# wafgo/rt-depth-map

Measured on AMD Instinct MI355X. Metric: stereo-pairs/sec, 1280x720 d=64 9x9 SAD, higher is better.
Workload: dtype u8

## Files before the change

rt-depth-map_amd/csrc/api_bm.hip:

```cpp
#include "rtdm_handles.h"

using namespace rtdm;

void rtdm_bm_default_params(rtdm_bm_params* p, int numDisparities)
{
    if (!p) return;
    p->preFilterCap = 31; p->blockSize = 13; p->minDisparity = 0; p->numDisparities = numDisparities;
    p->textureThreshold = 10; p->uniquenessRatio = 10; p->speckleWindowSize = 100; p->speckleRange = 32;
    p->disp12MaxDiff = 1; p->legacy_right_clamp = 0;
}

static int validate_params(const rtdm_bm_params& p)
{
    if (p.preFilterCap < 1 || p.preFilterCap > 63) return RTDM_ERR_BAD_PARAM;
    if (p.blockSize < 5 || p.blockSize > 255 || (p.blockSize & 1) == 0) return RTDM_ERR_BAD_PARAM;
    if (p.numDisparities <= 0 || p.numDisparities % 16 != 0) return RTDM_ERR_BAD_PARAM;
    if (p.textureThreshold < 0 || p.uniquenessRatio < 0) return RTDM_ERR_BAD_PARAM;
    if (p.minDisparity < -2047 || (long)p.minDisparity + p.numDisparities > 2047) return RTDM_ERR_BAD_PARAM;
    if (p.legacy_right_clamp != 0 && p.legacy_right_clamp != 1) return RTDM_ERR_BAD_PARAM;
    return RTDM_OK;
}

int rtdm_bm_create(const rtdm_bm_params* params, int max_width, int max_height, int max_batch,
                   int device, rtdm_bm** out)
{
    if (!params || !out) return RTDM_ERR_NULL;
    *out = nullptr;
    int rc = validate_params(*params);
    if (rc) return rc;
    if (max_width <= 0 || max_height <= 0 || max_batch <= 0 || max_width > 32767 || max_height > 32767)
        return RTDM_ERR_BAD_SIZE;
    if ((long)max_batch * max_width * max_height >= (1L << 31)) return RTDM_ERR_BAD_SIZE;
    if (max_width > 4096) return RTDM_ERR_UNSUPPORTED;
    rc = use_device(device);
    if (rc) return rc;
    rtdm_bm* bm = new (std::nothrow) rtdm_bm();
    if (!bm) return RTDM_ERR_NOMEM;
    bm->p = *params; bm->prefilter_type = RTDM_PREFILTER_XSOBEL; bm->prefilter_size = 9;
    bm->maxW = max_width; bm->maxH = max_height; bm->maxB = max_batch; bm->device = device;
    bm->ppitch = ((size_t)max_width + 63) & ~(size_t)63;
    const size_t plane = bm->ppitch * max_height * (size_t)max_batch;
    const size_t px = bm_ws(max_width) * max_height * max_batch;
    AllocList& m = bm->mem;
    m.err = hipStreamCreateWithFlags(&bm->stream, hipStreamNonBlocking);
    const size_t plane_al = (plane + 1024 + 255) & ~(size_t)255;
    if (m.dev(&bm->dLp, 2 * plane_al)) bm->dRp = bm->dLp + plane_al;
    m.dev(&bm->dInL, plane); m.dev(&bm->dInR, plane); m.dev(&bm->dOut, px * sizeof(int16_t));
    m.dev(&bm->dCost, px * sizeof(int32_t)); m.dev(&bm->dLabel, px * sizeof(int32_t)); m.dev(&bm->dSize, px * sizeof(int32_t));
    m.dev(&bm->dRuns, px * sizeof(uint32_t)); m.dev(&bm->dHead, px * sizeof(int16_t));
    m.dev(&bm->dMask, (size_t)max_width * max_height); m.dev(&bm->dDepth, depth_scratch_bytes(RTDM_MAX_REGIONS, max_height));
    const size_t hplanes = 2 * bm->ppitch * (size_t)max_height, hpx = bm_ws(max_width) * max_height;
    m.host(&bm->hStage, hplanes + hpx * (sizeof(int16_t) + 1) + 1024);
    if (bm->hStage) { bm->hD = (int16_t*)(bm->hStage + hplanes); bm->hM = (uint8_t*)(bm->hD + hpx); }
    m.dev(&bm->dRowCnt, (size_t)max_batch * max_height * sizeof(int32_t));
    hipError_t e = m.err;
    const auto new_event = [&e](hipEvent_t* ev) { if (e == hipSuccess) e = hipEventCreateWithFlags(ev, hipEventDisableTiming); };
    const auto new_stream = [&e](hipStream_t* q) { if (e == hipSuccess) e = hipStreamCreateWithFlags(q, hipStreamNonBlocking); };
    for (auto& ev : bm->evBand) new_event(&ev);
    new_stream(&bm->sIn); new_stream(&bm->sOut);
    for (int k = 0; k < 2; ++k) { new_event(&bm->evH2D[k]); new_event(&bm->evComp[k]); new_event(&bm->evD2H[k]); }
    new_stream(&bm->sSpare[0]); new_stream(&bm->sBorder); new_stream(&bm->sSpare[1]);
    new_event(&bm->evFork); new_event(&bm->evJoin);
    if (e != hipSuccess) { rtdm_bm_destroy(bm); return create_failed("rtdm_bm_create", e); }
    *out = bm;
    return RTDM_OK;
}

void rtdm_bm_destroy(rtdm_bm* bm)
{
    if (!bm) return;
    (void)hipSetDevice(bm->device);
    if (bm->stream) (void)hipStreamSynchronize(bm->stream);
    if (bm->sBorder) { (void)hipStreamSynchronize(bm->sBorder); (void)hipStreamDestroy(bm->sBorder); }
    for (auto& q : bm->sSpare) if (q) (void)hipStreamDestroy(q);
    for (hipEvent_t e : {bm->evFork, bm->evJoin, bm->evBand[0], bm->evBand[1]}) if (e) (void)hipEventDestroy(e);
    if (bm->sIn) { (void)hipStreamSynchronize(bm->sIn); (void)hipStreamDestroy(bm->sIn); }
    if (bm->sOut) { (void)hipStreamSynchronize(bm->sOut); (void)hipStreamDestroy(bm->sOut); }
    for (int k = 0; k < 2; ++k)
        for (hipEvent_t e : {bm->evH2D[k], bm->evComp[k], bm->evD2H[k]}) if (e) (void)hipEventDestroy(e);
    for (auto& ev : bm->pending) { (void)hipEventDestroy(ev.a); (void)hipEventDestroy(ev.b); }
    bm->mem.release();
    if (bm->stream) (void)hipStreamDestroy(bm->stream);
    delete bm;
}

int rtdm_bm_set_roi(rtdm_bm* bm, int which, int x, int y, int width, int height)
{
    if (!bm) return RTDM_ERR_NULL;
    if (which != 1 && which != 2) return RTDM_ERR_BAD_PARAM;
    int* r = which == 1 ? bm->roi1 : bm->roi2;
    r[0] = x; r[1] = y; r[2] = width; r[3] = height;
    return RTDM_OK;
}

int rtdm_bm_get_params(const rtdm_bm* bm, rtdm_bm_params* out)
{
    if (!bm || !out) return RTDM_ERR_NULL;
    *out = bm->p;
    return RTDM_OK;
}

int rtdm_bm_set_prefilter(rtdm_bm* bm, int preFilterType, int preFilterSize)
{
    if (!bm) return RTDM_ERR_NULL;
    if (preFilterType != RTDM_PREFILTER_NORMALIZED_RESPONSE && preFilterType != RTDM_PREFILTER_XSOBEL) return RTDM_ERR_BAD_PARAM;
    if (preFilterSize < 5 || preFilterSize > 255 || (preFilterSize & 1) == 0) return RTDM_ERR_BAD_PARAM;
    bm->prefilter_type = preFilterType; bm->prefilter_size = preFilterSize;
    return RTDM_OK;
}

int rtdm_bm_get_prefilter(const rtdm_bm* bm, int* preFilterType, int* preFilterSize)
{
    if (!bm || !preFilterType || !preFilterSize) return RTDM_ERR_NULL;
    *preFilterType = bm->prefilter_type; *preFilterSize = bm->prefilter_size;
    return RTDM_OK;
}

static bool make_geom(const rtdm_bm* bm, int W, int H, BMGeom* g)
{
    const rtdm_bm_params& p = bm->p;
    g->W = W; g->H = H; g->Ws = (W + 7) & ~7; g->D = p.numDisparities; g->minD = p.minDisparity;
    g->w = p.blockSize; g->r = p.blockSize / 2;
    g->cap = p.preFilterCap; g->tex = p.textureThreshold; g->uniq = p.uniquenessRatio;
    g->lofs = std::max(g->D - 1 + g->minD, 0);
    g->rofs = -std::min(g->D - 1 + g->minD, 0);
    g->width1 = W - g->rofs - g->D + 1;
    g->filtered = (g->minD - 1) * 16;
    g->want_cost = p.disp12MaxDiff >= 0;
    g->cost16 = 2L * p.preFilterCap * p.blockSize * p.blockSize < 65536;
    g->mask_cols = p.disp12MaxDiff < 0;
    g->legacy = p.legacy_right_clamp;
    int r1[4] = {0, 0, W, H}, r2[4] = {0, 0, W, H};
    if (bm->roi1[2] > 0 && bm->roi1[3] > 0) std::copy(bm->roi1, bm->roi1 + 4, r1);
    if (bm->roi2[2] > 0 && bm->roi2[3] > 0) std::copy(bm->roi2, bm->roi2 + 4, r2);
    const int maxD = g->minD + g->D - 1;
    int xmin = std::max(r1[0], r2[0] + maxD) + g->r;
    int xmax = std::min(r1[0] + r1[2], r2[0] + r2[2] - g->minD) - g->r;
    int ymin = std::max(r1[1], r2[1]) + g->r;
    int ymax = std::min(r1[1] + r1[3], r2[1] + r2[3]) - g->r;
    xmin = std::max(xmin, 0); xmax = std::min(xmax, W);
    ymin = std::max(ymin, g->r); ymax = std::min(ymax, H - g->r);
    g->vx0 = xmin; g->vx1 = xmax; g->vy0 = ymin; g->vy1 = ymax;
    const int reach = (p.disp12MaxDiff >= 0) ? g->D + std::abs(g->minD) + 2 : 0;
    g->cx0 = std::max(g->lofs, xmin - reach);
    g->cx1 = std::min(std::min(W, g->lofs + g->width1), xmax + reach);
    if (g->lofs >= W || g->rofs >= W || g->width1 < 1) return false;
    return xmax > xmin && ymax > ymin;
}

static void stage_begin(rtdm_bm* bm, int stage, int frames, hipStream_t s, StageEvent* ev)
{
    if (!bm->profiling) return;
    ev->stage = stage; ev->frames = frames;
    (void)hipEventCreate(&ev->a); (void)hipEventCreate(&ev->b);
    (void)hipEventRecord(ev->a, s);
}
static void stage_end(rtdm_bm* bm, hipStream_t s, StageEvent* ev)
{
    if (!bm->profiling) return;
    (void)hipEventRecord(ev->b, s);
    bm->pending.push_back(*ev);
}

static int chunk_front(rtdm_bm* bm, int n, Plane8 L, Plane8 R, int W, int H, Plane16W disp, hipStream_t s, BMGeom* gout,
                       bool* anyout)
{
    const rtdm_bm_params& p = bm->p;
    BMGeom& g = *gout;
    const bool any = make_geom(bm, W, H, &g);
    *anyout = any;
    if (!any) { launch_fill16(disp, 0, W, 0, H, n, g.filtered, s); return RTDM_OK; }
    const FillJob fill{disp, g.cx0, g.cx1, g.vy0, g.vy1, g.filtered, (p.speckleRange >= 0 && p.speckleWindowSize > 0) ? bm->dRowCnt : nullptr};
    StageEvent ev;
    Plane8W Lp{bm->dLp, bm->ppitch, bm->ppitch * (size_t)H}, Rp{bm->dRp, bm->ppitch, bm->ppitch * (size_t)H};
    stage_begin(bm, RTDM_STAGE_PREFILTER, n, s, &ev);
    launch_prefilter(L, R, Lp, Rp, W, H, p.preFilterCap, n, s, &fill, bm->prefilter_type, bm->prefilter_size);
    stage_end(bm, s, &ev);
    Plane8 Lpr{bm->dLp, Lp.pitch, Lp.frame}, Rpr{bm->dRp, Rp.pitch, Rp.frame};
    stage_begin(bm, RTDM_STAGE_SEARCH, n, s, &ev);
    const SearchPlan plan = plan_search(g, n, bm->dRp > bm->dLp && (size_t)(bm->dRp - bm->dLp) < ((size_t)1 << 32) - ((size_t)1 << 20));
    bm->variant = plan.variant;
    HIPC(launch_search(plan, Lpr, Rpr, disp, bm->dCost, g, n, s, SearchSide{bm->sBorder, bm->evFork, bm->evJoin}, &bm->tuner));
    stage_end(bm, s, &ev);
    HIPC(hipGetLastError());
    return RTDM_OK;
}

static int chunk_back(rtdm_bm* bm, int n, int W, int H, Plane16W disp, const BMGeom& g, hipStream_t s)
{
    const rtdm_bm_params& p = bm->p;
    StageEvent ev;
    const bool speckle = p.speckleRange >= 0 && p.speckleWindowSize > 0;
    const bool lr = p.disp12MaxDiff >= 0;
    int compact_rows = 0;
    if (lr) {
        stage_begin(bm, RTDM_STAGE_LRCHECK, n, s, &ev);
        if (speckle) compact_rows = launch_lrcheck(disp, bm->dCost, g, p.disp12MaxDiff, n, s, bm->dLabel, bm->dSize, bm->dRuns, bm->dRowCnt, bm->dHead,
                                                   p.speckleRange);
        else         launch_lrcheck(disp, bm->dCost, g, p.disp12MaxDiff, n, s);
        stage_end(bm, s, &ev);
    }
    if (speckle) {
        stage_begin(bm, RTDM_STAGE_SPECKLE, n, s, &ev);
        launch_speckle(disp, bm->dLabel, bm->dSize, bm->dRuns, bm->dRowCnt, bm->dHead, W, g.Ws, H, n, g.filtered, p.speckleWindowSize,
                       p.speckleRange, lr, std::max(compact_rows, 1), g.vy0, g.vy1, s, compact_rows > 0);
        stage_end(bm, s, &ev);
    }
    HIPC(hipGetLastError());
    return RTDM_OK;
}

int rtdm::bm_run_chunk(rtdm_bm* bm, int n, Plane8 L, Plane8 R, int W, int H, Plane16W out, hipStream_t s)
{
    const size_t Ws = bm_ws(W);
    const bool internal = out.pitch_e == Ws && out.base >= bm->dOut && out.base < bm->dOut + (size_t)bm->maxB * Ws * (size_t)H &&
                          (size_t)(out.base - bm->dOut) % (Ws * (size_t)H) == 0;
    const bool direct = internal || ((W & 7) == 0 && (((size_t)out.base | (out.pitch_e * 2) | (out.frame_e * 2)) & 15) == 0);
    const Plane16W disp = direct ? out : bm_internal_plane(bm, W, H);
    BMGeom g;
    bool any = false;
    int rc = chunk_front(bm, n, L, R, W, H, disp, s, &g, &any);
    if (rc) return rc;
    if (any) { rc = chunk_back(bm, n, W, H, disp, g, s); if (rc) return rc; }
    if (!direct) launch_copy16(disp, out, W, H, n, s);
    HIPC(hipGetLastError());
    return RTDM_OK;
}

int rtdm::bm_check_frame(const rtdm_bm* bm, int W, int H)
{
    if (W <= 0 || H <= 0 || W > bm->maxW || H > bm->maxH) return RTDM_ERR_BAD_SIZE;
    if (bm->p.blockSize >= std::min(W, H)) return RTDM_ERR_BAD_PARAM;
    return RTDM_OK;
}

int rtdm_bm_compute_device(rtdm_bm* bm, int n, const uint8_t* d_left, const uint8_t* d_right,
                           size_t pitch, size_t frame_stride, int width, int height,
                           int16_t* d_disp, size_t disp_pitch, size_t disp_frame_stride, void* hip_stream)
{
    if (!bm || !d_left || !d_right || !d_disp) return RTDM_ERR_NULL;
    if (n <= 0) return RTDM_ERR_BAD_SIZE;
    int rc = bm_check_frame(bm, width, height);
    if (rc) return rc;
    if (pitch < (size_t)width || disp_pitch < (size_t)width * 2 || (disp_pitch & 1) || (disp_frame_stride & 1))
        return RTDM_ERR_BAD_SIZE;
    HIPC(hipSetDevice(bm->device));
    hipStream_t s = (hipStream_t)hip_stream;
    for (int i0 = 0; i0 < n; i0 += bm->maxB) {
        const int m = std::min(bm->maxB, n - i0);
        Plane8 L{d_left + (size_t)i0 * frame_stride, pitch, frame_stride};
        Plane8 R{d_right + (size_t)i0 * frame_stride, pitch, frame_stride};
        Plane16W O{d_disp + (size_t)i0 * (disp_frame_stride / 2), disp_pitch / 2, disp_frame_stride / 2};
        rc = bm_run_chunk(bm, m, L, R, width, height, O, s);
        if (rc) return rc;
    }
    return RTDM_OK;
}

int rtdm_bm_compute_batch(rtdm_bm* bm, int n, const uint8_t* left, const uint8_t* right,
                          size_t pitch, size_t frame_stride, int width, int height,
                          int16_t* disp, size_t disp_pitch, size_t disp_frame_stride)
{
    if (!bm || !left || !right || !disp) return RTDM_ERR_NULL;
    if (n <= 0) return RTDM_ERR_BAD_SIZE;
    int rc = bm_check_frame(bm, width, height);
    if (rc) return rc;
    if (pitch < (size_t)width || disp_pitch < (size_t)width * 2) return RTDM_ERR_BAD_SIZE;
    HIPC(hipSetDevice(bm->device));
    hipStream_t s = bm->stream;
    DrainOnError drain(bm->sIn, s, bm->sOut);
    const size_t dpitch = bm->ppitch, dframe = bm->ppitch * (size_t)height;
    const size_t Ws = bm_ws(width);
    const size_t opitch = Ws * 2, oframe = opitch * (size_t)height;
    const int half = std::max(1, bm->maxB / 2);
    const bool two = bm->maxB >= 2 && page_locked(left) && page_locked(right) && page_locked(disp);
    const int chunk = two ? half : bm->maxB;
    int k = 0;
    for (int i0 = 0; i0 < n; i0 += chunk, ++k) {
        const int m = std::min(chunk, n - i0), b = two ? (k & 1) : 0;
        const size_t fo = (size_t)b * (size_t)half;
        hipStream_t si = two ? bm->sIn : s, so = two ? bm->sOut : s;
        if (two && k >= 2) HIPC(hipStreamWaitEvent(si, bm->evComp[b], 0));
        uint8_t *dl = bm->dInL + fo * dframe, *dr = bm->dInR + fo * dframe;
        if (pitch == dpitch && frame_stride == dframe) {
            const size_t nbytes = (size_t)m * dframe - (dpitch - (size_t)width);
            HIPC(hipMemcpyAsync(dl, left + (size_t)i0 * frame_stride, nbytes, hipMemcpyHostToDevice, si));
            HIPC(hipMemcpyAsync(dr, right + (size_t)i0 * frame_stride, nbytes, hipMemcpyHostToDevice, si));
        } else {
            for (int i = 0; i < m; ++i) {
                HIPC(hipMemcpy2DAsync(dl + i * dframe, dpitch, left + (size_t)(i0 + i) * frame_stride, pitch, width, height, hipMemcpyHostToDevice, si));
                HIPC(hipMemcpy2DAsync(dr + i * dframe, dpitch, right + (size_t)(i0 + i) * frame_stride, pitch, width, height, hipMemcpyHostToDevice, si));
            }
        }
        if (two) {
            HIPC(hipEventRecord(bm->evH2D[b], si));
            HIPC(hipStreamWaitEvent(s, bm->evH2D[b], 0));
            if (k >= 2) HIPC(hipStreamWaitEvent(s, bm->evD2H[b], 0));
        }
        Plane8 L{dl, dpitch, dframe}, R{dr, dpitch, dframe};
        int16_t* dout = bm->dOut + fo * Ws * (size_t)height;
        Plane16W O{dout, Ws, Ws * (size_t)height};
        rc = bm_run_chunk(bm, m, L, R, width, height, O, s);
        if (rc) return rc;
        if (two) { HIPC(hipEventRecord(bm->evComp[b], s)); HIPC(hipStreamWaitEvent(so, bm->evComp[b], 0)); }
        if ((size_t)width == Ws && disp_pitch == opitch && disp_frame_stride == oframe) {
            HIPC(hipMemcpyAsync((uint8_t*)disp + (size_t)i0 * disp_frame_stride, dout, (size_t)m * oframe, hipMemcpyDeviceToHost, so));
        } else {
            for (int i = 0; i < m; ++i)
                HIPC(hipMemcpy2DAsync((uint8_t*)disp + (size_t)(i0 + i) * disp_frame_stride, disp_pitch,
                                      (uint8_t*)dout + i * oframe, opitch, (size_t)width * 2, height, hipMemcpyDeviceToHost, so));
        }
        if (two) HIPC(hipEventRecord(bm->evD2H[b], so));
        else HIPC(hipStreamSynchronize(s));
    }
    if (two) { HIPC(hipStreamSynchronize(bm->sOut)); HIPC(hipStreamSynchronize(s)); HIPC(hipStreamSynchronize(bm->sIn)); }
    drain.armed = false;
    return RTDM_OK;
}

int rtdm_bm_compute(rtdm_bm* bm, const uint8_t* left, size_t left_pitch, const uint8_t* right,
                    size_t right_pitch, int width, int height, int16_t* disp, size_t disp_pitch)
{
    if (!bm || !left || !right || !disp) return RTDM_ERR_NULL;
    int rc = bm_check_frame(bm, width, height);
    if (rc) return rc;
    if (left_pitch < (size_t)width || right_pitch < (size_t)width || disp_pitch < (size_t)width * 2)
        return RTDM_ERR_BAD_SIZE;
    HIPC(hipSetDevice(bm->device));
    hipStream_t s = bm->stream;
    DrainOnError drain{s};
    const size_t dpitch = bm->ppitch, dframe = bm->ppitch * (size_t)height;
    const Plane16W O = bm_internal_plane(bm, width, height);
    const size_t Ws = O.pitch_e;
    if (page_locked(left) && page_locked(right) && page_locked(disp)) {
        HIPC(hipMemcpy2DAsync(bm->dInL, dpitch, left, left_pitch, (size_t)width, height, hipMemcpyHostToDevice, s));
        HIPC(hipMemcpy2DAsync(bm->dInR, dpitch, right, right_pitch, (size_t)width, height, hipMemcpyHostToDevice, s));
        Plane8 Ld{bm->dInL, dpitch, dframe}, Rd{bm->dInR, dpitch, dframe};
        rc = bm_run_chunk(bm, 1, Ld, Rd, width, height, O, s);
        if (rc) return rc;
        HIPC(hipMemcpy2DAsync(disp, disp_pitch, bm->dOut, Ws * sizeof(int16_t), (size_t)width * sizeof(int16_t), height, hipMemcpyDeviceToHost, s));
        HIPC(hipStreamSynchronize(s));
        drain.armed = false;
        return RTDM_OK;
    }
    uint8_t *hL = bm->hStage, *hR = hL + dframe;
    int16_t* hD = bm->hD;
    const int nb = height >= 256 ? 2 : 1, bh = (height + nb - 1) / nb;
    const auto gather = [&](uint8_t* dst, const uint8_t* src, size_t spitch, int y0, int y1) {
        if (spitch == dpitch) { memcpy(dst + (size_t)y0 * dpitch, src + (size_t)y0 * spitch, (size_t)(y1 - y0 - 1) * dpitch + (size_t)width); return; }
// ... 149 lines not shown
```

rt-depth-map_amd/csrc/k_search_ring.hip:

```cpp
#include "rtdm_select.h"
#include "rtdm_border.h"
#include "rtdm_border2.h"
#include "rtdm_search.h"

#include <cmath>
#include <cstdlib>
#include <type_traits>
#include <utility>

namespace rtdm {

struct RingGeom {
    int x0, nx;
    int rs;
    uint32_t lastmask;
    int tiles, strips;
    unsigned nitems;
    unsigned chunk;
    uint32_t rdelta;
    int rebase;
    unsigned nborder;
    int bgx, bgy;
    int b2;
};

__host__ __device__ constexpr int ring_rpg(int D, int LPP) { return D >= 96 ? 4 : LPP; }

template <int D, int WS, int LPP = 2>
struct RingCfg {
    static constexpr int RPG = ring_rpg(D, LPP);
    static constexpr bool SPLIT = LPP != 2 || D >= 48 || (D == 32 && (WS == 9 || WS == 5));
    static constexpr bool B64 = SPLIT && D == 64;
    using Rec = SelRecord<D, B64>;
    static constexpr int NP = (WS + 3) / 4;
    static constexpr int W1 = WS + 1;
    static constexpr int PPW = 64 / LPP;
    static constexpr int DL = D / LPP;
    static constexpr int NGL = DL / 4;
    static constexpr int NRL = DL / 2;
    static constexpr int NW = NGL + NP - 1;
    static constexpr int LWD = PPW + NP;
    static constexpr int RWD = PPW + D / 4 + NP;
    static constexpr int ITEMS = (LWD + RWD + 63) / 64;
    static constexpr int SLOT = ITEMS * 64;
    static constexpr int TRIP = (W1 % RPG == 0) ? W1 : (2 * W1 % RPG == 0) ? 2 * W1 : 4 * W1;
    static_assert(W1 % 2 == 0 && TRIP % RPG == 0 && TRIP % W1 == 0, "block sizes are odd");
    static constexpr bool STATIC_SLOTS = ITEMS == 1 && TRIP % 4 == 0;
    static constexpr int NSLOT = STATIC_SLOTS ? 4 : 3;
    static constexpr int STG = (NSLOT * SLOT + (W1 + RPG) * PPW / 2 + 3) & ~3;
    static constexpr int WAVE_LDS = STG + PPW * RPG * Rec::DWORDS;
    static constexpr int RING_REGS = W1 * NRL;
    static constexpr int W3_LIMIT = 112;
    static constexpr int WAVES = LPP >= 8 ? 2 : LPP == 4 ? (RING_REGS <= 80 ? 4 : (RING_REGS <= 96 && NRL <= 8) ? 3 : 2) : (RING_REGS <= 72 && NRL <= 8) ? 4 : RING_REGS <= W3_LIMIT ? 3 : 2;
    static constexpr int TILE = 4 * PPW;
    static constexpr bool FUSE_BORDER = WAVES < 4;
    static constexpr bool FUSE_BORDER2 = D <= 192;
    static constexpr bool ROW_PTRS = !(LPP == 2 && RING_REGS > 88 && WAVES == 3);
};

template <int D, int WS, int LPP, bool BORDER>
struct RingBounds { static constexpr int WAVES = BORDER && RingCfg<D, WS, LPP>::WAVES > 1 ? RingCfg<D, WS, LPP>::WAVES - 1 : RingCfg<D, WS, LPP>::WAVES; };

template <int D, int WS, int LPP = 2>
struct RingState { uint64_t P[RingCfg<D, WS, LPP>::W1][RingCfg<D, WS, LPP>::NGL]; };

template <int D, int WS, int LPP = 2>
struct RowRegs { uint64_t win[RingCfg<D, WS, LPP>::NW]; uint32_t l[RingCfg<D, WS, LPP>::NP]; };

typedef __attribute__((address_space(3))) const uint32_t* lds_cptr;
__device__ __forceinline__ uint32_t lds_addr(const uint32_t* q) { return (uint32_t)(uintptr_t)(lds_cptr)q; }
__device__ __forceinline__ lds_cptr lds_at(uint32_t a) { return (lds_cptr)(uintptr_t)a; }

template <int D, int WS, int LPP, typename PTR>
__device__ __forceinline__ void ring_load_row(PTR lp, PTR rp, PTR rpo, RowRegs<D, WS, LPP>& rw)
{
    using C = RingCfg<D, WS, LPP>;
#pragma unroll
    for (int k = 0; k < C::NP; ++k) rw.l[k] = lp[k];
#pragma unroll
    for (int j = 0; j < C::NW; ++j) {
        const PTR wp = (j & 1) ? rpo + (j - 1) : rp + j;
        rw.win[j] = (uint64_t)wp[0] | ((uint64_t)wp[1] << 32);
    }
}

template <int D, int WS, int LPP, int K, int NRLc>
__device__ __forceinline__ void ring_step(RingState<D, WS, LPP>& st, const RowRegs<D, WS, LPP>& rw, uint32_t lastmask, uint32_t capb,
                                          uint32_t& tnew, uint32_t (&S)[NRLc])
{
    using C = RingCfg<D, WS, LPP>;
    auto& P = st.P;
    constexpr int NP = C::NP, NGL = C::NGL, W1 = C::W1;
    constexpr int KP = (K + W1 - 1) % W1, KO = (K + 1) % W1;
    uint32_t l[NP];
#pragma unroll
    for (int k = 0; k < NP; ++k) l[k] = rw.l[k];
    l[NP - 1] &= lastmask;
#pragma unroll
    for (int k = 0; k < NP - 1; ++k) tnew = __builtin_amdgcn_sad_u8(l[k], capb, tnew);
    tnew = __builtin_amdgcn_msad_u8(capb, l[NP - 1], tnew);
#pragma unroll
    for (int j = 0; j < C::NW; ++j) {
#pragma unroll
        for (int k = 0; k < NP; ++k) {
            const int gi = j - k;
            if (gi >= 0 && gi < NGL) {
                const uint64_t acc = k == 0 ? P[KP][gi] : P[K][gi];
                if (k == NP - 1) P[K][gi] = __builtin_amdgcn_mqsad_pk_u16_u8(rw.win[j], l[k], acc);
                else             P[K][gi] = __builtin_amdgcn_qsad_pk_u16_u8(rw.win[j], l[k], acc);
            }
        }
    }
#pragma unroll
    for (int gi = 0; gi < NGL; ++gi) {
        S[2 * gi] = (uint32_t)P[K][gi] - (uint32_t)P[KO][gi];
        S[2 * gi + 1] = (uint32_t)(P[K][gi] >> 32) - (uint32_t)(P[KO][gi] >> 32);
    }
}

template <int N>
__device__ __forceinline__ void pin(uint32_t (&v)[N])
{
#pragma unroll
    for (int i = 0; i < N; ++i) asm volatile("" : "+v"(v[i]));
}

template <typename F, int... U>
__device__ __forceinline__ void ring_for_groups(std::integer_sequence<int, U...>, F&& f)
{ (void)(f(std::integral_constant<int, U>{}) && ...); }
template <typename F, int... R>
__device__ __forceinline__ void ring_for_rows(std::integer_sequence<int, R...>, F&& f)
{ (f(std::integral_constant<int, R>{}), ...); }

template <int D, int WS, int LPP, bool FUSE>
__global__ __launch_bounds__(256, (RingBounds<D, WS, LPP, FUSE>::WAVES)) void k_search_ring(Plane8 Lp, Plane8 Rp, Plane16W disp, uint16_t* cost, BMGeom g, RingGeom rg,
                                                                                   BorderGeom bg, Border2Geom b2g)
{
    using C = RingCfg<D, WS, LPP>;
    constexpr int NGL = C::NGL, NRL = C::NRL, W1 = C::W1, LWD = C::LWD, SLOT = C::SLOT, ITEMS = C::ITEMS, PPW = C::PPW, RPG = C::RPG;
    constexpr bool SPLIT = C::SPLIT;
    constexpr int RECD = C::Rec::DWORDS;
    extern __shared__ __attribute__((aligned(16))) uint32_t lds[];

    unsigned fi = blockIdx.x;
    if constexpr (FUSE) {
        if (fi < rg.nborder) {
            const unsigned per = (unsigned)(rg.bgx * rg.bgy), fr = fi / per, id = fi - fr * per;
            if (C::FUSE_BORDER2 && rg.b2) {
                const int wave = __builtin_amdgcn_readfirstlane((int)(threadIdx.x >> 6));
                border2_body<D, C::NP>(Lp, Rp, disp, cost, g, b2g, (int)(id % rg.bgx) * 4 + wave, (int)(id / rg.bgx), (int)fr);
            } else if constexpr (C::FUSE_BORDER) {
                border_body<(D + 63) / 64>((unsigned char*)lds, Lp, Rp, disp, cost, g, bg, (int)(id % rg.bgx), (int)(id / rg.bgx), (int)fr);
            }
            return;
        }
        fi -= rg.nborder;
    }
    if (rg.chunk) fi = (fi & 7u) * rg.chunk + (fi >> 3);
    if (fi >= rg.nitems) return;
    const int b_tile = (int)(fi % rg.tiles), b_strip = (int)((fi / rg.tiles) % rg.strips), f = (int)(fi / (rg.tiles * rg.strips));

    const int tid = threadIdx.x, lane = tid & 63;
    const int phi = __builtin_amdgcn_readfirstlane(tid >> 6);
    const int p = lane & (PPW - 1), h = lane / PPW;
    const int x_tile = rg.x0 + b_tile * C::TILE;
    const int x = x_tile + phi + 4 * p;
    const bool active = x < rg.x0 + rg.nx;
    const int ys0 = g.vy0 + b_strip * rg.rs;
    const int ys1 = min(ys0 + rg.rs, g.vy1);
    if (ys0 >= ys1) return;
    const int r = g.r;
    const uint8_t* Lb = Lp.base + (size_t)f * Lp.frame;
    const int Lbase = g.lofs + x_tile - r + phi;
    const int Rbase = g.rofs + x_tile - r + phi;
    const uint32_t capb = (uint32_t)(g.cap + PREFILTER_BIAS) * 0x01010101u;

    uint32_t* stg = lds + phi * C::WAVE_LDS;
    unsigned short* ptr = (unsigned short*)(stg + C::NSLOT * SLOT);
    unsigned short* ptw = ptr + W1 * PPW;
    const bool owner = RPG == LPP || h < RPG;
    const unsigned short* ptw_own = ptw + (owner ? h : 0) * PPW + p;
    uint32_t* scr = stg + C::STG + (owner ? lane : 0) * RECD;
    uint32_t* scr_w = stg + C::STG + p * RECD + h * NRL;
    using GSel = GroupSelectRec<D, LPP, C::B64>;
    unsigned short* scr_m = (unsigned short*)(stg + C::STG + p * RECD + D / 2) + h * (NRL / 4);
    if constexpr (SPLIT) GSel::init(scr);

    const int row0 = ys0 - r;
    const int Hm1 = g.H - 1;
    const uint8_t* rowp = Lb + (size_t)row0 * Lp.pitch;
    uint32_t loff[ITEMS];
#pragma unroll
    for (int it = 0; it < ITEMS; ++it) {
        const int idx = lane + it * 64;
        const bool isr = idx >= LWD;
        const int m = isr ? idx - LWD : idx;
        loff[it] = (uint32_t)((isr ? Rbase : Lbase) + 4 * m) + (isr ? rg.rdelta : 0u);
    }
    int next_row = row0;
    uint32_t pre[2][ITEMS];
    auto issue = [&](auto Sc) {
        constexpr int SET = decltype(Sc)::value;
#pragma unroll
        for (int it = 0; it < ITEMS; ++it) {
            asm volatile("" : "+v"(loff[it]));
            pre[SET][it] = *(const uint32_t*)(rowp + loff[it]);
        }
        rowp += next_row < Hm1 ? Lp.pitch : 0;
        ++next_row;
    };
    auto commit = [&](auto Sc, auto slot) {
        constexpr int SET = decltype(Sc)::value;
#pragma unroll
        for (int it = 0; it < ITEMS; ++it) stg[slot * SLOT + lane + it * 64] = pre[SET][it];
        __builtin_amdgcn_wave_barrier();
    };
    using Set0 = std::integral_constant<int, 0>;
    using Set1 = std::integral_constant<int, 1>;

    RingState<D, WS, LPP> st;
#pragma unroll
    for (int k = 0; k < W1; ++k)
#pragma unroll
        for (int i = 0; i < NGL; ++i) st.P[k][i] = 0;
#pragma unroll
    for (int k = 0; k < W1; ++k) ptr[k * PPW + p] = 0;
    uint32_t pt = 0;

    const int nsteps = (ys1 - ys0) + WS - 1;
    const int nstepsg = (nsteps + RPG - 1) / RPG * RPG;
    issue(Set0{}); issue(Set1{});
    commit(Set0{}, 0); commit(Set1{}, 1);
    issue(Set0{});

    char* const db = (char*)(disp.base + (size_t)f * disp.frame_e);
    char* const cb = (char*)(cost + (size_t)f * g.H * g.Ws);
    const int col = g.lofs + x;
    constexpr int TF = (WS - 1) / RPG * RPG;
    uint32_t dofs = (uint32_t)(((long long)(ys0 + TF + h - (WS - 1)) * (long long)disp.pitch_e + col) * 2);
    uint32_t cofs = (uint32_t)(((long long)(ys0 + TF + h - (WS - 1)) * (long long)g.Ws + col) * 2);
    const uint32_t dstep = (uint32_t)(disp.pitch_e * 2 * RPG), cstep = (uint32_t)(g.Ws * 2 * RPG);
    const bool masked_col = g.mask_cols && (col < g.vx0 || col >= g.vx1);

    uint32_t S[RPG][NRL];
    int sl_cur = 0;
    uint32_t la_cur = lds_addr(stg + p), ra_cur = lds_addr(stg + LWD + p + h * NGL), ro_cur = ra_cur + 4;
    if constexpr (C::STATIC_SLOTS) asm volatile("" : "+v"(la_cur), "+v"(ra_cur), "+v"(ro_cur));
    const auto lds_row = [&](auto SLc, RowRegs<D, WS, LPP>& rw) {
        if constexpr (C::STATIC_SLOTS) {
            constexpr uint32_t off = (uint32_t)(decltype(SLc)::value * SLOT * 4);
            ring_load_row<D, WS, LPP>(lds_at(la_cur + off), lds_at(ra_cur + off), lds_at(ro_cur + off), rw);
        } else if constexpr (C::ROW_PTRS) {
            asm volatile("" : "+v"(la_cur), "+v"(ra_cur), "+v"(ro_cur));
            ring_load_row<D, WS, LPP>(lds_at(la_cur), lds_at(ra_cur), lds_at(ro_cur), rw);
            const uint32_t adv = (uint32_t)((sl_cur == 2 ? -2 * SLOT : SLOT) * 4);
            la_cur += adv; ra_cur += adv; ro_cur += adv;
        } else {
            int li = sl_cur * SLOT + p, ri = sl_cur * SLOT + LWD + p + h * NGL, one = 1;
            asm volatile("" : "+v"(li), "+v"(ri), "+v"(one));
            ring_load_row<D, WS, LPP, const uint32_t*>(stg + li, stg + ri, stg + ri + one, rw);
        }
    };
    auto step = [&](auto Kc, auto SLc, auto Rc, const RowRegs<D, WS, LPP>& rw, uint32_t (&Sr)[NRL]) {
        constexpr int K = decltype(Kc)::value;
        using SetIn = std::integral_constant<int, (K + 1) & 1>;
        using SetOut = std::integral_constant<int, K & 1>;
        issue(SetIn{});
        uint32_t tnew = 0;
        ring_step<D, WS, LPP, K>(st, rw, rg.lastmask, capb, tnew, Sr);
        constexpr int KO = (K + 1) % W1;
        pt += tnew;
        const uint32_t told = ptr[KO * PPW + p];
        ptr[K * PPW + p] = (unsigned short)pt;
        ptw[decltype(Rc)::value * PPW + p] = (unsigned short)(pt - told);
        pin(Sr);
        if constexpr (C::STATIC_SLOTS) {
            commit(SetOut{}, std::integral_constant<int, (decltype(SLc)::value + 2) % 4>{});
        } else {
            const int sl_new = sl_cur == 0 ? 2 : sl_cur - 1;
            sl_cur = sl_cur == 2 ? 0 : sl_cur + 1;
            commit(SetOut{}, sl_new);
        }
    };

    int trips_since_rebase = 0;
    for (int t0 = 0; t0 < nstepsg; t0 += C::TRIP) {
        if (rg.rebase && ++trips_since_rebase > rg.rebase) {
            trips_since_rebase = 1;
#pragma unroll
            for (int i = 0; i < NGL; ++i) {
                const uint32_t blo = (uint32_t)st.P[1][i], bhi = (uint32_t)(st.P[1][i] >> 32);
#pragma unroll
                for (int k = 1; k < W1; ++k) {
                    const uint32_t lo = (uint32_t)st.P[k][i] - blo, hi = (uint32_t)(st.P[k][i] >> 32) - bhi;
                    st.P[k][i] = (uint64_t)lo | ((uint64_t)hi << 32);
                }
            }
        }
        ring_for_groups(std::make_integer_sequence<int, C::TRIP / RPG>{}, [&](auto Uc) -> bool {
            constexpr int U = RPG * decltype(Uc)::value;
            const int t = t0 + U;
            if (t >= nstepsg) return false;
            GSel gsel;
            ring_for_rows(std::make_integer_sequence<int, RPG>{}, [&](auto Rc) {
                constexpr int R = decltype(Rc)::value;
                RowRegs<D, WS, LPP> rw;
                using SL = std::integral_constant<int, (U + R) % 4>;
                lds_row(SL{}, rw);
                step(std::integral_constant<int, (U + R) % W1>{}, SL{}, Rc, rw, S[R]);
                if constexpr (SPLIT) gsel.template row<R>(S[R], scr_w + R * (PPW * RECD), scr_m + R * (PPW * RECD * 2));
            });
            if (t + RPG - 1 < WS - 1) return true;
            const int y = ys0 + (t - (WS - 1)) + h;
            const bool row_ok = owner && y >= ys0 && y < ys1;
            const uint32_t dof = dofs, cof = cofs;
            dofs += dstep; cofs += cstep;
            const int tsum = *ptw_own;
            const bool dead = !active | !row_ok | masked_col | (tsum < g.tex);
            if (__builtin_amdgcn_ballot_w64(!dead) == 0) {
                if (active && row_ok) *(int16_t*)(db + dof) = (int16_t)g.filtered;
            } else {
                int m1; bool fail;
                int out;
                if constexpr (SPLIT) {
                    int uq = g.uniq;
                    asm volatile("" : "+s"(uq));
                    out = gsel.finish(tsum, g, uq > 0, scr, &m1, &fail);
                } else {
                    uint32_t rr[D / 2];
#pragma unroll
                    for (int i = 0; i < NRL; ++i) {
                        const auto sw = __builtin_amdgcn_permlane32_swap(S[0][i], S[RPG - 1][i], false, false);
                        rr[i] = sw[0]; rr[NRL + i] = sw[1];
                    }
                    out = select_disparity_lds<D>(rr, tsum, g, scr, &m1, &fail);
                }
                if (active && row_ok) {
                    if (!fail && g.want_cost) *(uint16_t*)(cb + cof) = (uint16_t)m1;
                    *(int16_t*)(db + dof) = (int16_t)(masked_col ? g.filtered : out);
                }
            }
            return true;
        });
    }
}


static int ring_rows_cap(const BMGeom& g) { return 65535 / (g.w * 2 * g.cap) - g.w - 6; }
static int ring_rebase_trips(const BMGeom& g, int lpp)
{
    const int W1 = g.w + 1, rpg = ring_rpg(g.D, lpp);
    const int trip = (W1 % rpg == 0) ? W1 : (2 * W1 % rpg == 0) ? 2 * W1 : 4 * W1;
    return ring_rows_cap(g) / trip;
}
static int ring_min_strips(const BMGeom& g, int lpp, int nrows)
{ return ring_rebase_trips(g, lpp) > 0 ? 1 : max(1, (nrows + ring_rows_cap(g) - 1) / ring_rows_cap(g)); }

#ifdef RTDM_RING_DEV
#define RTDM_RING_TABLE(X) RTDM_RING_DEV
#else
#define RTDM_RING_TABLE(X) X(64, 9, 2) X(64, 7, 2) X(64, 5, 2) X(32, 7, 2) X(32, 9, 2) X(32, 11, 2) X(32, 13, 2) X(48, 7, 2) X(48, 9, 2) \
                           X(16, 5, 2) X(16, 7, 2) X(16, 9, 2) X(64, 9, 4) X(64, 7, 4) X(64, 5, 4) X(64, 11, 4) X(64, 13, 4) \
                           X(128, 7, 8) X(128, 9, 8) X(128, 11, 8) X(128, 13, 8) X(96, 7, 4) X(96, 9, 4) X(96, 11, 4) X(96, 13, 4) X(48, 11, 2) X(48, 13, 2) \
                           X(16, 11, 2) X(16, 13, 2) X(32, 5, 2) X(32, 15, 2) X(48, 5, 2) X(64, 15, 4) X(128, 15, 8) \
                           X(192, 9, 8) X(192, 11, 8) X(192, 13, 8) X(192, 15, 8) X(256, 9, 16) X(256, 11, 16) X(256, 13, 16) X(256, 15, 16)
#endif

static std::atomic<int> g_ring_switch{0};
void ring_set_mode(int mode)
{
    const int m = mode < 0 ? -1 : mode == 0 ? 0 : 1, lpp = (mode == 2 || mode == 4 || mode == 8) ? mode : 0;
    g_ring_switch.store((m + 1) | (lpp << 8), std::memory_order_relaxed);
}
static int ring_mode() { return (g_ring_switch.load(std::memory_order_relaxed) & 0xff) - 1; }
static int ring_forced_lpp() { return g_ring_switch.load(std::memory_order_relaxed) >> 8; }

static int ring_lpp(const BMGeom& g)
{
    int have = 0;
#define X(DD, WW, LL) if (g.D == DD && g.w == WW) have |= LL;
    RTDM_RING_TABLE(X)
#undef X
    const int want = ring_forced_lpp();
    if (want && (have & want) == want) return want;
    return (have & 16) ? 16 : (have & 8) ? 8 : (have & 4) ? 4 : (have & 2) ? 2 : 0;
}

static RingForm ring_form_of(const BMGeom& g, int lpp)
{
#define X(DD, WW, LL) if (g.D == DD && g.w == WW && lpp == LL) { using C = RingCfg<DD, WW, LL>; return RingForm{LL, C::WAVES, C::FUSE_BORDER2, C::FUSE_BORDER, C::TILE}; }
    RTDM_RING_TABLE(X)
#undef X
    return RingForm{};
}

RingForm ring_form(const BMGeom& g)
{
    const RingForm none{};
    if (ring_mode() == 0) return none;
    if (2L * g.cap * g.w * g.w > 32766) return none;
    if (2L * g.cap * g.w * g.w >= 0x7C00) return none;
    if (ring_rows_cap(g) < 2) return none;
    if ((size_t)g.H * (size_t)g.Ws * 2 >= ((size_t)1 << 32)) return none;
    return ring_form_of(g, ring_lpp(g));
}

int ring_strips_model(const SearchPlan& plan, const BMGeom& g, int n)
{
    const int tile = 256 / plan.lanes, tiles = (plan.nx + tile - 1) / tile, nrows = g.vy1 - g.vy0;
    const int slots = 256 * ring_form_of(g, plan.lanes).waves;
    const int smin = ring_min_strips(g, plan.lanes, nrows), smax = max(smin, (nrows + 15) / 16);
    const float fill = 0.5f * (float)(g.w - 1);
    int s = (int)(sqrtf((float)nrows * (float)slots / (fill * (float)tiles * (float)n)) + 0.5f);
    s = max(smin, min(s, smax));
    if ((long)tiles * s * n < 6L * slots) {
        float best = 1e30f;
        for (int c = smin; c <= smax; ++c) {
            const int rs = (nrows + c - 1) / c, ce = (nrows + rs - 1) / rs;
            const long rounds = ((long)tiles * ce * n + slots - 1) / slots;
            const float t = (float)rounds * ((float)rs + fill + 2.0f);
            if (t < best) { best = t; s = ce; }
        }
    }
    return s;
}

template <int D, int WS, int LPP>
static void ring_launch_one(const SearchPlan& plan, Plane8 Lp, Plane8 Rp, Plane16W disp, void* cost, const BMGeom& g, int n, hipStream_t stream,
                            int strips_hint)
{
    using C = RingCfg<D, WS, LPP>;
    RingGeom rg;
    rg.rdelta = (uint32_t)(Rp.base - Lp.base);
    rg.x0 = plan.x0; rg.nx = plan.nx;
    const int rem = g.w - 4 * (C::NP - 1);
    rg.lastmask = rem >= 4 ? 0xffffffffu : ((1u << (8 * rem)) - 1u);
    const int nrows = g.vy1 - g.vy0;
    const int tiles = (rg.nx + C::TILE - 1) / C::TILE;
    int strips = strips_hint > 0 ? strips_hint : ring_strips_model(plan, g, n);
    strips = max(strips, ring_min_strips(g, LPP, nrows));
    rg.rebase = ring_rebase_trips(g, LPP);
    strips = max(1, min(strips, nrows));
    rg.rs = (nrows + strips - 1) / strips;
    strips = (nrows + rg.rs - 1) / rg.rs;
    rg.tiles = tiles; rg.strips = strips;
    rg.nitems = (unsigned)tiles * strips * n;
    rg.chunk = (rg.nitems + 7) / 8;
    const unsigned grid = rg.chunk * 8;
    BorderGeom bg{};
    Border2Geom b2g{};
    size_t blds = 0;
    rg.nborder = 0; rg.bgx = rg.bgy = 0; rg.b2 = 0;
    if (plan.place == BorderPlace::FUSED && plan.border.form != BorderForm::NONE) {
        const BorderPlan& b = plan.border;
        if (b.form == BorderForm::ROWS) { b2g = b.rows; rg.b2 = 1; }
        else { bg = b.disp; blds = b.lds; }
        rg.bgx = b.gx; rg.bgy = b.gy;
        rg.nborder = (unsigned)(rg.bgx * rg.bgy) * (unsigned)n;
    }
    const size_t ldsb = max((size_t)4 * C::WAVE_LDS * sizeof(uint32_t), blds);
    const auto launch = [&](auto Fc) {
        constexpr bool F = decltype(Fc)::value;
        constexpr size_t ring_lds = (size_t)4 * C::WAVE_LDS * sizeof(uint32_t);
        const size_t most = C::FUSE_BORDER ? max(ring_lds, border_lds_bytes(D, WS)) : ring_lds;
        static OncePerDevice once;
        if (most > 48 * 1024 && once.first()) {
            int dev = 0, lds_max = 0;
            size_t want = max(most, (size_t)64 * 1024);
            if (hipGetDevice(&dev) == hipSuccess &&
                hipDeviceGetAttribute(&lds_max, hipDeviceAttributeMaxSharedMemoryPerMultiprocessor, dev) == hipSuccess && lds_max > 0)
                want = min(want, (size_t)lds_max);
            (void)hipGetLastError();
            (void)hipFuncSetAttribute((const void*)k_search_ring<D, WS, LPP, F>, hipFuncAttributeMaxDynamicSharedMemorySize, (int)want);
        }
        hipLaunchKernelGGL((k_search_ring<D, WS, LPP, F>), dim3(grid + rg.nborder), dim3(256), ldsb, stream, Lp, Rp, disp, (uint16_t*)cost, g, rg, bg, b2g);
    };
    if (rg.nborder) launch(std::true_type{});
    else launch(std::false_type{});
}

void launch_search_ring(const SearchPlan& plan, Plane8 Lp, Plane8 Rp, Plane16W disp, void* cost, const BMGeom& g, int n, hipStream_t stream,
                        int strips)
{
#define X(DD, WW, LL) if (g.D == DD && g.w == WW && plan.lanes == LL) { ring_launch_one<DD, WW, LL>(plan, Lp, Rp, disp, cost, g, n, stream, strips); return; }
    RTDM_RING_TABLE(X)
#undef X
}

}
```

Baseline: 73300.

## Pair adjacent columns per lane to share SAD window dwords in ring search

For D=64, 9x9 windows with four lanes per pixel, each lane now computes costs for two neighbouring columns whose 9-wide windows overlap. The shared middle dwords are summed once with qsad and only the edge bytes differ, handled by mqsad. This roughly halves the SAD instruction work per column. It costs a second ring state of registers, fixes the kernel at three waves, disables the fused border pass, and changes the LDS record layout. The left/right plane pointer also gets a 256-byte front pad so the shifted loads stay inside the allocation.

```diff
diff --git a/rt-depth-map_amd/csrc/api_bm.hip b/rt-depth-map_amd/csrc/api_bm.hip
--- a/rt-depth-map_amd/csrc/api_bm.hip
+++ b/rt-depth-map_amd/csrc/api_bm.hip
@@ -43,8 +43,8 @@
     const size_t px = bm_ws(max_width) * max_height * max_batch;
     AllocList& m = bm->mem;
     m.err = hipStreamCreateWithFlags(&bm->stream, hipStreamNonBlocking);
-    const size_t plane_al = (plane + 1024 + 255) & ~(size_t)255;
-    if (m.dev(&bm->dLp, 2 * plane_al)) bm->dRp = bm->dLp + plane_al;
+    const size_t plane_al = (plane + 1024 + 255) & ~(size_t)255, front = 256;
+    if (m.dev(&bm->dLp, front + 2 * plane_al)) { bm->dLp += front; bm->dRp = bm->dLp + plane_al; }
     m.dev(&bm->dInL, plane); m.dev(&bm->dInR, plane); m.dev(&bm->dOut, px * sizeof(int16_t));
     m.dev(&bm->dCost, px * sizeof(int32_t)); m.dev(&bm->dLabel, px * sizeof(int32_t)); m.dev(&bm->dSize, px * sizeof(int32_t));
     m.dev(&bm->dRuns, px * sizeof(uint32_t)); m.dev(&bm->dHead, px * sizeof(int16_t));
diff --git a/rt-depth-map_amd/csrc/k_search_ring.hip b/rt-depth-map_amd/csrc/k_search_ring.hip
--- a/rt-depth-map_amd/csrc/k_search_ring.hip
+++ b/rt-depth-map_amd/csrc/k_search_ring.hip
@@ -35,12 +35,16 @@
     static constexpr int NP = (WS + 3) / 4;
     static constexpr int W1 = WS + 1;
     static constexpr int PPW = 64 / LPP;
-    static constexpr int DL = D / LPP;
+    static constexpr bool PAIR = D == 64 && WS == 9 && LPP == 4;
+    static constexpr int LPG = PAIR ? 2 * LPP : LPP;
+    static constexpr int GPW = 64 / LPG;
+    static constexpr int DL = D / LPG;
     static constexpr int NGL = DL / 4;
     static constexpr int NRL = DL / 2;
-    static constexpr int NW = NGL + NP - 1;
-    static constexpr int LWD = PPW + NP;
-    static constexpr int RWD = PPW + D / 4 + NP;
+    static constexpr int NL = PAIR ? NP + 1 : NP;
+    static constexpr int NW = NGL + NL - 1;
+    static constexpr int LWD = GPW + NP;
+    static constexpr int RWD = GPW + D / 4 + NP;
     static constexpr int ITEMS = (LWD + RWD + 63) / 64;
     static constexpr int SLOT = ITEMS * 64;
     static constexpr int TRIP = (W1 % RPG == 0) ? W1 : (2 * W1 % RPG == 0) ? 2 * W1 : 4 * W1;
@@ -48,24 +52,34 @@
     static constexpr bool STATIC_SLOTS = ITEMS == 1 && TRIP % 4 == 0;
     static constexpr int NSLOT = STATIC_SLOTS ? 4 : 3;
     static constexpr int STG = (NSLOT * SLOT + (W1 + RPG) * PPW / 2 + 3) & ~3;
-    static constexpr int WAVE_LDS = STG + PPW * RPG * Rec::DWORDS;
-    static constexpr int RING_REGS = W1 * NRL;
+    static constexpr int PREC = D / 2 + D / 16;
+    static constexpr int PREC_PAIR = LPG * PREC;
+    __host__ __device__ static constexpr int pair_rec(int p, int o) { return p * PREC_PAIR + o * PREC + 2 * (p & 1) + 8 * (p >> 1); }
+    static constexpr int REC_DWORDS = PAIR ? pair_rec(GPW - 1, LPG - 1) + PREC + 2 : PPW * RPG * Rec::DWORDS;
+    static constexpr int WAVE_LDS = STG + REC_DWORDS;
+    static constexpr int RING_REGS = W1 * NRL * (PAIR ? 2 : 1);
     static constexpr int W3_LIMIT = 112;
-    static constexpr int WAVES = LPP >= 8 ? 2 : LPP == 4 ? (RING_REGS <= 80 ? 4 : (RING_REGS <= 96 && NRL <= 8) ? 3 : 2) : (RING_REGS <= 72 && NRL <= 8) ? 4 : RING_REGS <= W3_LIMIT ? 3 : 2;
+    static constexpr int WAVES = PAIR ? 3 : LPP >= 8 ? 2 : LPP == 4 ? (RING_REGS <= 80 ? 4 : (RING_REGS <= 96 && NRL <= 8) ? 3 : 2) : (RING_REGS <= 72 && NRL <= 8) ? 4 : RING_REGS <= W3_LIMIT ? 3 : 2;
     static constexpr int TILE = 4 * PPW;
-    static constexpr bool FUSE_BORDER = WAVES < 4;
+    static constexpr bool FUSE_BORDER = WAVES < 4 && !PAIR;
     static constexpr bool FUSE_BORDER2 = D <= 192;
     static constexpr bool ROW_PTRS = !(LPP == 2 && RING_REGS > 88 && WAVES == 3);
 };
 
 template <int D, int WS, int LPP, bool BORDER>
-struct RingBounds { static constexpr int WAVES = BORDER && RingCfg<D, WS, LPP>::WAVES > 1 ? RingCfg<D, WS, LPP>::WAVES - 1 : RingCfg<D, WS, LPP>::WAVES; };
+struct RingBounds {
+    using C = RingCfg<D, WS, LPP>;
+    static constexpr int WAVES = BORDER && C::WAVES > 1 && !C::PAIR ? C::WAVES - 1 : C::WAVES;
+};
 
 template <int D, int WS, int LPP = 2>
-struct RingState { uint64_t P[RingCfg<D, WS, LPP>::W1][RingCfg<D, WS, LPP>::NGL]; };
+struct RingState {
+    uint64_t P[RingCfg<D, WS, LPP>::W1][RingCfg<D, WS, LPP>::NGL];
+    uint64_t P2[RingCfg<D, WS, LPP>::PAIR ? RingCfg<D, WS, LPP>::W1 : 1][RingCfg<D, WS, LPP>::NGL];
+};
 
 template <int D, int WS, int LPP = 2>
-struct RowRegs { uint64_t win[RingCfg<D, WS, LPP>::NW]; uint32_t l[RingCfg<D, WS, LPP>::NP]; };
+struct RowRegs { uint64_t win[RingCfg<D, WS, LPP>::NW]; uint32_t l[RingCfg<D, WS, LPP>::NL]; };
 
 typedef __attribute__((address_space(3))) const uint32_t* lds_cptr;
 __device__ __forceinline__ uint32_t lds_addr(const uint32_t* q) { return (uint32_t)(uintptr_t)(lds_cptr)q; }
@@ -76,7 +90,7 @@
 {
     using C = RingCfg<D, WS, LPP>;
 #pragma unroll
-    for (int k = 0; k < C::NP; ++k) rw.l[k] = lp[k];
+    for (int k = 0; k < C::NL; ++k) rw.l[k] = lp[k];
 #pragma unroll
     for (int j = 0; j < C::NW; ++j) {
         const PTR wp = (j & 1) ? rpo + (j - 1) : rp + j;
@@ -118,6 +132,50 @@
     }
 }
 
+__device__ __forceinline__ uint64_t ring_add_halves(uint64_t a, uint64_t b)
+{
+    typedef uint32_t u2 __attribute__((ext_vector_type(2)));
+    return __builtin_bit_cast(uint64_t, __builtin_bit_cast(u2, a) + __builtin_bit_cast(u2, b));
+}
+
+template <int D, int WS, int LPP, int K, int NRLc>
+__device__ __forceinline__ void ring_step_pair(RingState<D, WS, LPP>& st, const RowRegs<D, WS, LPP>& rw, uint32_t capb,
+                                               uint32_t& tpk, uint32_t (&S)[NRLc], uint32_t (&S2)[NRLc])
+{
+    using C = RingCfg<D, WS, LPP>;
+    static_assert(C::PAIR && WS % 4 == 1, "the two windows share whole dwords only for w = 1 (mod 4)");
+    constexpr int NP = C::NP, NGL = C::NGL, W1 = C::W1;
+    constexpr int KP = (K + W1 - 1) % W1, KO = (K + 1) % W1;
+    const uint32_t lf = rw.l[0] & 0xff000000u, ll = rw.l[NP] & 0x000000ffu;
+    uint32_t tsh = 0;
+#pragma unroll
+    for (int k = 1; k < NP; ++k) tsh = __builtin_amdgcn_sad_u8(rw.l[k], capb, tsh);
+    const uint32_t t1 = __builtin_amdgcn_msad_u8(capb, lf, tsh), t2 = __builtin_amdgcn_msad_u8(capb, ll, tsh);
+    tpk = t1 | (t2 << 16);
+    uint64_t sh[NGL], e1[NGL], e2[NGL];
+#pragma unroll
+    for (int j = 0; j < C::NW; ++j) {
+#pragma unroll
+        for (int k = 0; k <= NP; ++k) {
+            const int gi = j - k;
+            if (gi >= 0 && gi < NGL) {
+                if (k == 0)       e1[gi] = __builtin_amdgcn_mqsad_pk_u16_u8(rw.win[j], lf, st.P[KP][gi]);
+                else if (k == NP) e2[gi] = __builtin_amdgcn_mqsad_pk_u16_u8(rw.win[j], ll, st.P2[KP][gi]);
+                else              sh[gi] = __builtin_amdgcn_qsad_pk_u16_u8(rw.win[j], rw.l[k], k == 1 ? (uint64_t)0 : sh[gi]);
+            }
+        }
+    }
+#pragma unroll
+    for (int gi = 0; gi < NGL; ++gi) {
+        st.P[K][gi] = ring_add_halves(e1[gi], sh[gi]);
+        st.P2[K][gi] = ring_add_halves(e2[gi], sh[gi]);
+        S[2 * gi] = (uint32_t)st.P[K][gi] - (uint32_t)st.P[KO][gi];
+        S[2 * gi + 1] = (uint32_t)(st.P[K][gi] >> 32) - (uint32_t)(st.P[KO][gi] >> 32);
+        S2[2 * gi] = (uint32_t)st.P2[K][gi] - (uint32_t)st.P2[KO][gi];
+        S2[2 * gi + 1] = (uint32_t)(st.P2[K][gi] >> 32) - (uint32_t)(st.P2[KO][gi] >> 32);
+    }
+}
+
 template <int N>
 __device__ __forceinline__ void pin(uint32_t (&v)[N])
 {
@@ -138,7 +196,9 @@
 {
     using C = RingCfg<D, WS, LPP>;
     constexpr int NGL = C::NGL, NRL = C::NRL, W1 = C::W1, LWD = C::LWD, SLOT = C::SLOT, ITEMS = C::ITEMS, PPW = C::PPW, RPG = C::RPG;
-    constexpr bool SPLIT = C::SPLIT;
+    constexpr int GPW = C::GPW;
+    constexpr bool SPLIT = C::SPLIT, PAIR = C::PAIR;
+    static_assert(!PAIR || (SPLIT && C::STATIC_SLOTS && C::LPG == 2 * RPG), "the paired layout: one owner lane per (column, row) of a group");
     constexpr int RECD = C::Rec::DWORDS;
     extern __shared__ __attribute__((aligned(16))) uint32_t lds[];
 
@@ -162,39 +222,45 @@
 
     const int tid = threadIdx.x, lane = tid & 63;
     const int phi = __builtin_amdgcn_readfirstlane(tid >> 6);
-    const int p = lane & (PPW - 1), h = lane / PPW;
+    const int p = lane & (GPW - 1), h = lane / GPW;
     const int x_tile = rg.x0 + b_tile * C::TILE;
-    const int x = x_tile + phi + 4 * p;
+    const int xw = PAIR ? x_tile + (phi >> 1) * (C::TILE / 2) + 2 * (phi & 1) : x_tile + phi;
+    const int hrow = PAIR ? h >> 1 : h;
+    const int x = xw + 4 * p + (PAIR ? h & 1 : 0);
     const bool active = x < rg.x0 + rg.nx;
     const int ys0 = g.vy0 + b_strip * rg.rs;
     const int ys1 = min(ys0 + rg.rs, g.vy1);
     if (ys0 >= ys1) return;
     const int r = g.r;
     const uint8_t* Lb = Lp.base + (size_t)f * Lp.frame;
-    const int Lbase = g.lofs + x_tile - r + phi;
-    const int Rbase = g.rofs + x_tile - r + phi;
+    constexpr int PAIR_SHIFT = PAIR ? 3 : 0;
+    const int Lbase = g.lofs + xw - r;
+    const int Rbase = g.rofs + xw - r;
     const uint32_t capb = (uint32_t)(g.cap + PREFILTER_BIAS) * 0x01010101u;
 
     uint32_t* stg = lds + phi * C::WAVE_LDS;
     unsigned short* ptr = (unsigned short*)(stg + C::NSLOT * SLOT);
     unsigned short* ptw = ptr + W1 * PPW;
-    const bool owner = RPG == LPP || h < RPG;
-    const unsigned short* ptw_own = ptw + (owner ? h : 0) * PPW + p;
-    uint32_t* scr = stg + C::STG + (owner ? lane : 0) * RECD;
-    uint32_t* scr_w = stg + C::STG + p * RECD + h * NRL;
-    using GSel = GroupSelectRec<D, LPP, C::B64>;
-    unsigned short* scr_m = (unsigned short*)(stg + C::STG + p * RECD + D / 2) + h * (NRL / 4);
+    uint32_t* const ptr2 = (uint32_t*)ptr;
+    uint32_t* const ptw2 = (uint32_t*)ptw;
+    const bool owner = PAIR || RPG == LPP || h < RPG;
+    const unsigned short* ptw_own = ptw + (owner ? hrow : 0) * PPW + (PAIR ? 2 * p + (h & 1) : p);
+    uint32_t* scr = stg + C::STG + (PAIR ? C::pair_rec(p, h) : (owner ? lane : 0) * RECD);
+    uint32_t* const rec0 = stg + C::STG + (PAIR ? C::pair_rec(p, 0) : p * RECD);
+    uint32_t* scr_w = rec0 + h * NRL;
+    using GSel = GroupSelectRec<D, C::LPG, C::B64>;
+    unsigned short* scr_m = (unsigned short*)(rec0 + D / 2) + h * (NRL / 4);
     if constexpr (SPLIT) GSel::init(scr);
 
     const int row0 = ys0 - r;
     const int Hm1 = g.H - 1;
-    const uint8_t* rowp = Lb + (size_t)row0 * Lp.pitch;
+    const uint8_t* rowp = Lb + (size_t)row0 * Lp.pitch - PAIR_SHIFT;
     uint32_t loff[ITEMS];
 #pragma unroll
     for (int it = 0; it < ITEMS; ++it) {
         const int idx = lane + it * 64;
         const bool isr = idx >= LWD;
-        const int m = isr ? idx - LWD : idx;
+        const int m = isr ? (PAIR ? min(idx - LWD, C::RWD - 1) : idx - LWD) : idx;
         loff[it] = (uint32_t)((isr ? Rbase : Lbase) + 4 * m) + (isr ? rg.rdelta : 0u);
     }
     int next_row = row0;
@@ -222,9 +288,15 @@
 #pragma unroll
     for (int k = 0; k < W1; ++k)
 #pragma unroll
-        for (int i = 0; i < NGL; ++i) st.P[k][i] = 0;
-#pragma unroll
-    for (int k = 0; k < W1; ++k) ptr[k * PPW + p] = 0;
+        for (int i = 0; i < NGL; ++i) {
+            st.P[k][i] = 0;
+            if constexpr (PAIR) st.P2[k][i] = 0;
+        }
+#pragma unroll
+    for (int k = 0; k < W1; ++k) {
+        if constexpr (PAIR) ptr2[k * GPW + p] = 0;
+        else ptr[k * PPW + p] = 0;
+    }
     uint32_t pt = 0;
 
     const int nsteps = (ys1 - ys0) + WS - 1;
@@ -237,8 +309,8 @@
     char* const cb = (char*)(cost + (size_t)f * g.H * g.Ws);
     const int col = g.lofs + x;
     constexpr int TF = (WS - 1) / RPG * RPG;
-    uint32_t dofs = (uint32_t)(((long long)(ys0 + TF + h - (WS - 1)) * (long long)disp.pitch_e + col) * 2);
-    uint32_t cofs = (uint32_t)(((long long)(ys0 + TF + h - (WS - 1)) * (long long)g.Ws + col) * 2);
+    uint32_t dofs = (uint32_t)(((long long)(ys0 + TF + hrow - (WS - 1)) * (long long)disp.pitch_e + col) * 2);
+    uint32_t cofs = (uint32_t)(((long long)(ys0 + TF + hrow - (WS - 1)) * (long long)g.Ws + col) * 2);
     const uint32_t dstep = (uint32_t)(disp.pitch_e * 2 * RPG), cstep = (uint32_t)(g.Ws * 2 * RPG);
     const bool masked_col = g.mask_cols && (col < g.vx0 || col >= g.vx1);
 
@@ -261,18 +333,27 @@
             ring_load_row<D, WS, LPP, const uint32_t*>(stg + li, stg + ri, stg + ri + one, rw);
         }
     };
-    auto step = [&](auto Kc, auto SLc, auto Rc, const RowRegs<D, WS, LPP>& rw, uint32_t (&Sr)[NRL]) {
+    auto step = [&](auto Kc, auto SLc, auto Rc, const RowRegs<D, WS, LPP>& rw, uint32_t (&Sr)[NRL], uint32_t (&Sr2)[NRL]) {
         constexpr int K = decltype(Kc)::value;
         using SetIn = std::integral_constant<int, (K + 1) & 1>;
         using SetOut = std::integral_constant<int, K & 1>;
         issue(SetIn{});
         uint32_t tnew = 0;
-        ring_step<D, WS, LPP, K>(st, rw, rg.lastmask, capb, tnew, Sr);
         constexpr int KO = (K + 1) % W1;
-        pt += tnew;
-        const uint32_t told = ptr[KO * PPW + p];
-        ptr[K * PPW + p] = (unsigned short)pt;
-        ptw[decltype(Rc)::value * PPW + p] = (unsigned short)(pt - told);
+        if constexpr (PAIR) {
+            ring_step_pair<D, WS, LPP, K>(st, rw, capb, tnew, Sr, Sr2);
+            pt = __builtin_bit_cast(uint32_t, __builtin_bit_cast(sel_us2, pt) + __builtin_bit_cast(sel_us2, tnew));
+            const uint32_t told = ptr2[KO * GPW + p];
+            ptr2[K * GPW + p] = pt;
+            ptw2[decltype(Rc)::value * GPW + p] = __builtin_bit_cast(uint32_t, __builtin_bit_cast(sel_us2, pt) - __builtin_bit_cast(sel_us2, told));
+            pin(Sr2);
+        } else {
+            ring_step<D, WS, LPP, K>(st, rw, rg.lastmask, capb, tnew, Sr);
+            pt += tnew;
+            const uint32_t told = ptr[KO * PPW + p];
+            ptr[K * PPW + p] = (unsigned short)pt;
+            ptw[decltype(Rc)::value * PPW + p] = (unsigned short)(pt - told);
+        }
         pin(Sr);
         if constexpr (C::STATIC_SLOTS) {
             commit(SetOut{}, std::integral_constant<int, (decltype(SLc)::value + 2) % 4>{});
@@ -294,6 +375,14 @@
                 for (int k = 1; k < W1; ++k) {
                     const uint32_t lo = (uint32_t)st.P[k][i] - blo, hi = (uint32_t)(st.P[k][i] >> 32) - bhi;
                     st.P[k][i] = (uint64_t)lo | ((uint64_t)hi << 32);
+                }
+                if constexpr (PAIR) {
+                    const uint32_t blo2 = (uint32_t)st.P2[1][i], bhi2 = (uint32_t)(st.P2[1][i] >> 32);
+#pragma unroll
+                    for (int k = 1; k < W1; ++k) {
+                        const uint32_t lo = (uint32_t)st.P2[k][i] - blo2, hi = (uint32_t)(st.P2[k][i] >> 32) - bhi2;
+                        st.P2[k][i] = (uint64_t)lo | ((uint64_t)hi << 32);
+                    }
                 }
             }
         }
@@ -307,11 +396,15 @@
                 RowRegs<D, WS, LPP> rw;
                 using SL = std::integral_constant<int, (U + R) % 4>;
                 lds_row(SL{}, rw);
-                step(std::integral_constant<int, (U + R) % W1>{}, SL{}, Rc, rw, S[R]);
-                if constexpr (SPLIT) gsel.template row<R>(S[R], scr_w + R * (PPW * RECD), scr_m + R * (PPW * RECD * 2));
+                uint32_t S2[NRL] = {};
+                step(std::integral_constant<int, (U + R) % W1>{}, SL{}, Rc, rw, S[R], S2);
+                if constexpr (PAIR) {
+                    gsel.template row<R>(S[R], scr_w + 2 * R * C::PREC, scr_m + 2 * R * (C::PREC * 2));
+                    gsel.template row<R>(S2, scr_w + (2 * R + 1) * C::PREC, scr_m + (2 * R + 1) * (C::PREC * 2));
+                } else if constexpr (SPLIT) gsel.template row<R>(S[R], scr_w + R * (PPW * RECD), scr_m + R * (PPW * RECD * 2));
             });
             if (t + RPG - 1 < WS - 1) return true;
-            const int y = ys0 + (t - (WS - 1)) + h;
+            const int y = ys0 + (t - (WS - 1)) + hrow;
             const bool row_ok = owner && y >= ys0 && y < ys1;
             const uint32_t dof = dofs, cof = cofs;
             dofs += dstep; cofs += cstep;
```

Measured after the change: 74840, median of 6. 2.1% higher.
